# rvl-lab-utoronto/video_similarity_search

Measured on AMD Instinct MI355X. Metric: clips/sec R3D-18+NCE (1/2/4/8 GPU); k-means embeddings/sec 100k×512, higher is better.
Workload: dtype f32; 1 GPU; R3D-18 (3D-ResNet-18, 34.52 M params, no maxpool, 7^3 stem) fwd+bwd + NT-Xent (noise_contrastive, T=0.5) + SGD(lr .1, mom .5); per-GPU batch 32 x 3x16x112x112 fp32 = 16 anchors || 16 positives; BASELINE configs[1]; global_batch=32, parallelism=dp1

## Files before the change

include/slic_hip.h:

```cpp
#ifndef SLIC_HIP_H
#define SLIC_HIP_H

#include <stddef.h>
#include <stdint.h>

#ifdef __cplusplus
extern "C" {
#endif

#define SLIC_OK 0
#define SLIC_EINVAL -1
#define SLIC_EHIP -2
#define SLIC_ENODEV -3
#define SLIC_ETIMEOUT -4

int slic_version(void);
const char* slic_last_error(void);
int slic_device_check(void);


int slic_kmeans_cnorm(const float* C, int K, int D, int ldc, float* cnorm, void* stream);

size_t slic_kmeans_assign_workspace_bytes(int64_t N, int K);
int slic_kmeans_assign(const float* X, int64_t N, int D, int ldx, const float* C, int K, int ldc,
// ... 131 lines not shown
int slic_conv_gemm(const SlicConvArgs* args, int variant, void* stream);
int slic_conv_gemm_multi(const SlicConvArgs* args, int n, int variant, void* stream);
size_t slic_conv_gemm_tailsplit_workspace_bytes(const SlicConvArgs* args, int variant, int nfull_rb, int splits);
int slic_conv_gemm_tailsplit(const SlicConvArgs* args, int variant, int nfull_rb, int splits, void* workspace, void* stream);

size_t slic_conv_wgrad_workspace_bytes(const SlicConvArgs* args, int splits);
int slic_conv_wgrad(const SlicConvArgs* args, const float* dy, int ldy, int splits, int C, int ntaps,
                    float* dW, void* workspace, void* stream);
int slic_conv_row_table(const SlicConvArgs* args, uint32_t* row_tab, void* stream);
int slic_pack_weight_fwd(const float* W, int N, int C, int ntaps, int Cs, int Kp, float* Wp, void* stream);
int slic_pack_weight_fwd_runs(const float* W, int N, int C, int ntaps, int run_len, int run_px, int Kp, float* Wp, void* stream);
int slic_pack_weight_dgrad(const float* W, int N, int C, int ntaps, int Cs, int Kd, float* Wd, void* stream);
int slic_pack_weight_wino(const float* W, int N, int C, int dgrad, float* U, void* stream);
int slic_pack_weight_wino2(const float* W, int N, int C, int dgrad, float* U, void* stream);
size_t slic_conv_wgrad_wino2_workspace_bytes(const SlicConvArgs* args, int splits);
int slic_conv_wino2_tile_table(const SlicConvArgs* args, uint32_t* tile_tab, void* stream);
int slic_conv_wgrad_wino2(const SlicConvArgs* args, const float* dy, int splits, const uint32_t* tile_tab, float* dW,
                          void* workspace, void* stream);
size_t slic_conv_wgrad_wino_workspace_bytes(const SlicConvArgs* args, int splits);
int slic_conv_wino_tile_table(const SlicConvArgs* args, uint32_t* tile_tab, void* stream);
int slic_conv_wgrad_wino(const SlicConvArgs* args, const float* dy, int splits, const uint32_t* tile_tab, float* dW,
                         void* workspace, void* stream);
int slic_ncdhw_to_ndhwc(const float* x, int B, int C, int64_t S, int Cp, float* y, void* stream);
int slic_ncdhw_to_ndhwc_wpad(const float* x, int B, int C, int64_t R, int W, int pad_left, int Wp, float* y, void* stream);

int slic_pack_weight_stem_dgrad(const float* W, int N, int C, int kt, float* Wp, void* stream);
int slic_conv_stem_dgrad(const float* dz, const float* Wp, int B, int C, int T, int H, int W, int N, int kt, int st, float* dx,
                         void* stream);

int slic_bn_merge_stats(const float* partial, int R, int rows, int C, int64_t M, double* stats, void* workspace, void* stream);
// ... 174 lines not shown
```

video_similarity_search_amd/_lib.py:

```python
import ctypes
import os

import torch

_HERE = os.path.dirname(os.path.abspath(__file__))
LIB_PATH = os.environ.get("SLIC_LIB_PATH") or os.path.join(_HERE, "csrc", "libslic_hip.so")

c_void_p, c_int, c_int64, c_size_t, c_float, c_double = (
    ctypes.c_void_p, ctypes.c_int, ctypes.c_int64, ctypes.c_size_t, ctypes.c_float, ctypes.c_double)
P, I, L, F, Dbl = c_void_p, c_int, c_int64, c_float, c_double

SIGNATURES = {
    "slic_version": (I, []),
    "slic_last_error": (ctypes.c_char_p, []),
    "slic_device_check": (I, []),
    "slic_kmeans_cnorm": (I, [P, I, I, I, P, P]),
    "slic_kmeans_assign_workspace_bytes": (c_size_t, [L, I]),
    "slic_kmeans_assign": (I, [P, L, I, I, P, I, I, P, P, P, P, P, P, P]),
    "slic_kmeans_accumulate_workspace_bytes": (c_size_t, [L, I]),
    "slic_kmeans_accumulate": (I, [P, L, I, I, P, I, P, P, P, P]),
    "slic_kmeans_combine_shards": (I, [P, P, L, I, I, I, P, P, P]),
    "slic_kmeans_dist_to_assigned": (I, [P, L, I, I, P, I, P, P, P]),
    "slic_sum_f32_to_f64_workspace_bytes": (c_size_t, [L]),
    "slic_sum_f32_to_f64": (I, [P, L, P, P, P]),
# ... 36 lines not shown
    "slic_cumsum_search": (I, [P, L, P, I, P, P, P]),
    "slic_conv_tile_m": (I, [P, I]),
    "slic_conv_gemm": (I, [P, I, P]),
    "slic_conv_gemm_multi": (I, [P, I, I, P]),
    "slic_conv_gemm_tailsplit_workspace_bytes": (c_size_t, [P, I, I, I]),
    "slic_conv_gemm_tailsplit": (I, [P, I, I, I, P, P]),
    "slic_conv_wgrad_workspace_bytes": (c_size_t, [P, I]),
    "slic_conv_row_table": (I, [P, P, P]),
    "slic_conv_wgrad": (I, [P, P, I, I, I, I, P, P, P]),
    "slic_pack_weight_fwd": (I, [P, I, I, I, I, I, P, P]),
    "slic_pack_weight_fwd_runs": (I, [P, I, I, I, I, I, I, P, P]),
    "slic_pack_weight_dgrad": (I, [P, I, I, I, I, I, P, P]),
    "slic_pack_weight_wino": (I, [P, I, I, I, P, P]),
    "slic_pack_weight_wino2": (I, [P, I, I, I, P, P]),
    "slic_conv_wgrad_wino2_workspace_bytes": (c_size_t, [P, I]),
    "slic_conv_wino2_tile_table": (I, [P, P, P]),
    "slic_conv_wgrad_wino2": (I, [P, P, I, P, P, P, P]),
    "slic_conv_wgrad_wino_workspace_bytes": (c_size_t, [P, I]),
    "slic_conv_wino_tile_table": (I, [P, P, P]),
    "slic_conv_wgrad_wino": (I, [P, P, I, P, P, P, P]),
    "slic_ncdhw_to_ndhwc": (I, [P, I, I, L, I, P, P]),
    "slic_ncdhw_to_ndhwc_wpad": (I, [P, I, I, L, I, I, I, P, P]),
    "slic_pack_weight_stem_dgrad": (I, [P, I, I, I, P, P]),
    "slic_conv_stem_dgrad": (I, [P, P, I, I, I, I, I, I, I, I, P, P]),
    "slic_bn_finalize_workspace_bytes": (c_size_t, [I, I]),
    "slic_bn_finalize": (I, [P, I, I, I, L, F, F, P, P, P, P, P, P, P, P, P, P]),
    "slic_bn_eval_affine": (I, [P, P, P, P, F, I, P, P, P]),
    "slic_bn_merge_stats": (I, [P, I, I, I, L, P, P, P]),
    "slic_bn_finalize_sync": (I, [P, I, I, F, F, P, P, P, P, P, P, P, P, P]),
    "slic_bn_bwd_sums_workspace_bytes": (c_size_t, [L, I, I]),
# ... 175 lines not shown
```

video_similarity_search_amd/csrc/common.h:

```cpp
#pragma once
#include <hip/hip_runtime.h>
#include <stdint.h>
#include <stdio.h>
#include "../../include/slic_hip.h"

typedef float f32x4 __attribute__((ext_vector_type(4)));
typedef float f32x16 __attribute__((ext_vector_type(16)));
typedef int i32x4 __attribute__((ext_vector_type(4)));

void slic_set_error(const char* fmt, ...);

#define SLIC_REQUIRE(cond, ...)                 \
  do {                                          \
    if (!(cond)) {                              \
      slic_set_error(__VA_ARGS__);              \
      return SLIC_EINVAL;                       \
    }                                           \
  } while (0)

#define SLIC_HIP_CHECK(expr)                                                        \
  do {                                                                              \
    hipError_t _e = (expr);                                                         \
    if (_e != hipSuccess) {                                                         \
      slic_set_error("%s:%d: %s -> %s", __FILE__, __LINE__, #expr, hipGetErrorString(_e)); \
      return SLIC_EHIP;                                                             \
    }                                                                               \
  } while (0)

#define SLIC_LAUNCH_CHECK() SLIC_HIP_CHECK(hipGetLastError())

int slic_lds_limit(const void* kernel, size_t bytes);
int slic_device_cus(void);

#define SLIC_LDS_LIMIT(kernel, bytes)                                  \
  do {                                                                 \
    int _rc = slic_lds_limit((const void*)(kernel), (size_t)(bytes));  \
    if (_rc != SLIC_OK) return _rc;                                    \
  } while (0)

static inline hipStream_t S_(void* s) { return (hipStream_t)s; }

static inline size_t slic_align_up(size_t x, size_t a) { return (x + a - 1) / a * a; }
static inline int64_t slic_cdiv(int64_t a, int64_t b) { return (a + b - 1) / b; }

struct SlicCarver {
  char* p;
  size_t off;
// ... 9 lines not shown
```

video_similarity_search_amd/csrc/common.hip:

```cpp
#include "common.h"
#include <stdarg.h>
#include <string.h>
#include <map>
#include <mutex>
#include <utility>

static thread_local char g_err[512] = "";

void slic_set_error(const char* fmt, ...) {
  va_list ap;
  va_start(ap, fmt);
  vsnprintf(g_err, sizeof(g_err), fmt, ap);
  va_end(ap);
}

extern "C" int slic_version(void) { return (0 << 16) | (1 << 8) | 0; }

extern "C" const char* slic_last_error(void) { return g_err; }

extern "C" int slic_device_check(void) {
  int dev = 0;
  hipDeviceProp_t prop;
  if (hipGetDevice(&dev) != hipSuccess || hipGetDeviceProperties(&prop, dev) != hipSuccess) {
    slic_set_error("no HIP device visible");
// ... 14 lines not shown
  if (bytes > 160 * 1024) {
    slic_set_error("slic_lds_limit: %zu bytes of dynamic LDS", bytes);
    return SLIC_EHIP;
  }
  int dev = 0;
  SLIC_HIP_CHECK(hipGetDevice(&dev));
  std::lock_guard<std::mutex> lock(g_dev_mu);
  const auto key = std::make_pair(dev, kernel);
  const auto it = g_lds_limit.find(key);
  if (it != g_lds_limit.end() && bytes <= it->second) return SLIC_OK;
  SLIC_HIP_CHECK(hipFuncSetAttribute(kernel, hipFuncAttributeMaxDynamicSharedMemorySize, (int)bytes));
  g_lds_limit[key] = bytes;
  return SLIC_OK;
}

int slic_device_cus(void) {
  int dev = 0, cus = 0;
  if (hipGetDevice(&dev) != hipSuccess) { (void)hipGetLastError(); return 0; }
  std::lock_guard<std::mutex> lock(g_dev_mu);
  auto it = g_cus.find(dev);
  if (it != g_cus.end()) return it->second;
  if (hipDeviceGetAttribute(&cus, hipDeviceAttributeMultiprocessorCount, dev) != hipSuccess || cus <= 0) { (void)hipGetLastError(); return 0; }
  g_cus[dev] = cus;
  return cus;
}
```

video_similarity_search_amd/csrc/conv.hip:

```cpp
#include "common.h"
#include "conv_common.h"
#include "conv_internal.h"
#include <type_traits>
#ifndef SLIC_WG_ILVQ
#define SLIC_WG_ILVQ 7
#endif
#ifndef SLIC_PRIO_EDGE
#define SLIC_PRIO_EDGE 3
#endif
#ifndef SLIC_ILVQ
#define SLIC_ILVQ 2
#endif
#include <stdlib.h>
#ifndef SLIC_GEMM0_WPE
#define SLIC_GEMM0_WPE 4
#endif

#ifdef SLIC_STAMPS
__device__ unsigned long long* slic_stamps_buf = nullptr;
extern "C" int slic_debug_set_stamps(unsigned long long* buf) {
  return hipMemcpyToSymbol(HIP_SYMBOL(slic_stamps_buf), &buf, sizeof(buf)) == hipSuccess ? 0 : -1;
}
#define SLIC_STAMP(wg, slot)                                                                              \
  do {                                                                                                   \
// ... 22 lines not shown
    const int n = n0 + col;
    const float bias = (p.bias && n < p.N) ? p.bias[n] : 0.f;
#pragma unroll
    for (int i = 0; i < TM; ++i)
#pragma unroll
      for (int g = 0; g < 16; ++g) {
        const int row = wm * WTM + i * 32 + (g & 3) + 8 * (g >> 2) + 4 * h;
        tile[row * BN + col] = acc[i][j][g] + bias;
      }
  }
  __syncthreads();
  conv_epilogue_rows<BM, BN>(p, lds, m0, n0, tid);
}

template <int BM, int BN, int WM, int WN>
__global__ __launch_bounds__(256) __attribute__((amdgpu_waves_per_eu(SLIC_GEMM0_WPE, SLIC_GEMM0_WPE))) void conv_gemm_kernel(const SlicConvArgs p) {
  extern __shared__ __attribute__((aligned(16))) float lds[];
  constexpr int WTM = BM / WM, WTN = BN / WN;
  constexpr int TM = WTM / 32, TN = WTN / 32;
  constexpr int AL = BM / 32, BL = BN / 32;
  static_assert(WM * WN == 4, "4 waves");
  float* As = lds;
  float* Bs = lds + 2 * BM * 32;

  const int tid = threadIdx.x, lane = tid & 63, wave = tid >> 6;
  const int wm = wave / WN, wn = wave % WN;
  const int64_t m0 = (int64_t)blockIdx.x * BM;
  const int n0 = blockIdx.y * BN;

  const int cq = tid & 7, srow = tid >> 3;
  const __amdgpu_buffer_rsrc_t rs_src = __builtin_amdgcn_make_buffer_rsrc((void*)p.src, 0, p.src_bytes, 0x00020000);
// ... 17 lines not shown
      for (int o = -3; o <= 3; ++o) {
        mk |= ((unsigned)(a0 + o) < (unsigned)p.Ts ? 1u : 0u) << (o + 3);
        mk |= ((unsigned)(b0 + o) < (unsigned)p.Hs ? 1u : 0u) << (7 + o + 3);
        mk |= ((unsigned)(c0 + o) < (unsigned)p.Ws ? 1u : 0u) << (14 + o + 3);
      }
      rmask[i] = mk;
    }
  }
  unsigned woff[BL];
#pragma unroll
  for (int i = 0; i < BL; ++i) {
    const int n = n0 + srow + 32 * i;
    woff[i] = n < p.N ? (unsigned)n * (unsigned)p.ldw * 4u : OOB;
  }
  i32x4 gA[2][AL], gB[2][BL];
  const int nk = p.nchunks >> 3;
  int4 e_next = nk > 0 ? ((const int4*)p.tab)[cq] : make_int4(0, -1, 0, 0);
  auto gload = [&](int kt, i32x4 (&ga)[AL], i32x4 (&gb)[BL]) {
    const int4 e = e_next;
    const unsigned tm = (unsigned)e.y;
    const unsigned dlt = (unsigned)e.x * 4u;
#pragma unroll
    for (int i = 0; i < AL; ++i) {
      const unsigned off = ((rmask[i] & tm) == tm) ? aoff[i] + dlt : OOB;
      ga[i] = __builtin_amdgcn_raw_buffer_load_b128(rs_src, (int)off, 0, 0);
    }
    const unsigned wc = e.y == -1 ? OOB : (unsigned)e.z * 4u;
#pragma unroll
    for (int i = 0; i < BL; ++i) {
      const unsigned off = (woff[i] == OOB || wc == OOB) ? OOB : woff[i] + wc;
      gb[i] = __builtin_amdgcn_raw_buffer_load_b128(rs_wgt, (int)off, 0, 0);
    }
// ... 31 lines not shown
        for (int i = 0; i < TM; ++i) a[nxt][i] = *(const f32x4*)&Ab[cv_off(wm * WTM + i * 32 + r, 2 * (q + 1) + h)];
#pragma unroll
        for (int j = 0; j < TN; ++j) b[nxt][j] = *(const f32x4*)&Bb[cv_off(wn * WTN + j * 32 + r, 2 * (q + 1) + h)];
      }
#pragma unroll
      for (int t = 0; t < 4; ++t)
#pragma unroll
        for (int i = 0; i < TM; ++i)
#pragma unroll
          for (int j = 0; j < TN; ++j)
            acc[i][j] = __builtin_amdgcn_mfma_f32_32x32x2f32(a[cur][i][t], b[cur][j][t], acc[i][j], 0, 0, 0);
      if (q < 3) __builtin_amdgcn_sched_group_barrier(0x100, TM + TN, 0);
      __builtin_amdgcn_sched_group_barrier(0x008, 4 * TM * TN, 0);
    }
  };
  if (nk > 0) {
    gload(0, gA[0], gB[0]);
    lwrite(0, gA[0], gB[0]);
    if (nk > 1) gload(1, gA[1], gB[1]);
  }
  __syncthreads();
  for (int kt0 = 0; kt0 < nk; kt0 += 2) {
#pragma unroll
    for (int half = 0; half < 2; ++half) {
      const int kt = kt0 + half;
      if (kt < nk) {
        if (kt + 2 < nk) gload(kt + 2, gA[half], gB[half]);
        compute(half);
        if (kt + 1 < nk) lwrite(half ^ 1, gA[half ^ 1], gB[half ^ 1]);
        __syncthreads();
      }
    }
  }

  conv_epilogue<BM, BN, WM, WN, TM, TN>(p, acc, lds, m0, n0, wm, wn, r, h, tid);
}

// ... 1226 lines not shown
  }
  if (a->dst)
    SLIC_REQUIRE(a->N % 4 == 0 && a->ldo % 4 == 0 && ((uintptr_t)a->dst % 16) == 0 && (!a->addend || ((uintptr_t)a->addend % 16) == 0),
                 "%s: N and ldo must be multiples of 4 and dst / addend 16-byte aligned", who);
  SLIC_REQUIRE(((uintptr_t)a->src % 16) == 0, "%s: src not 16-byte aligned", who);
  SLIC_REQUIRE(a->src_bytes > 0 && a->src_bytes < 0xFFFFFF00u, "%s: src_bytes must be set and < 4 GiB (split the batch)", who);
  return SLIC_OK;
}

template <int BM, int BN, int WM, int WN>
static int launch_gemm(const SlicConvArgs& a, hipStream_t st) {
  constexpr size_t ring = (size_t)2 * (BM + BN) * 32 * sizeof(float), epi = (size_t)conv_epi_lds_floats(BM, BN) * sizeof(float);
  constexpr size_t lds = ring > epi ? ring : epi;
  SLIC_LDS_LIMIT((conv_gemm_kernel<BM, BN, WM, WN>), lds);
  dim3 grid((unsigned)slic_cdiv(a.M, BM), (unsigned)slic_cdiv(a.N, BN));
  conv_gemm_kernel<BM, BN, WM, WN><<<grid, dim3(256), lds, st>>>(a);
  SLIC_LAUNCH_CHECK();
  return SLIC_OK;
}

template <int BM, int BN, int WM, int WN, int STAGES = 2, int KD = 32>
static int launch_gemm_dma(const SlicConvArgs& a, hipStream_t st) {
  constexpr size_t ring = (size_t)STAGES * (BM + BN) * KD * sizeof(float), epi = (size_t)conv_epi_lds_floats(BM, BN) * sizeof(float);
  constexpr size_t lds = ring > epi ? ring : epi;
  SLIC_LDS_LIMIT((conv_gemm_dma_kernel<BM, BN, WM, WN, STAGES, KD>), lds);
  const unsigned gx = (unsigned)slic_cdiv(a.M, BM);
  dim3 grid((gx + 7) / 8 * 8, (unsigned)slic_cdiv(a.N, BN));
  conv_gemm_dma_kernel<BM, BN, WM, WN, STAGES, KD><<<grid, dim3(256), lds, st>>>(a, 1, nullptr, 0);
  SLIC_LAUNCH_CHECK();
  return SLIC_OK;
}
// ... 321 lines not shown
```

video_similarity_search_amd/csrc/conv_wino2.hip:

```cpp
#include "common.h"
#include "conv_epilogue.h"
#include "conv_internal.h"
#include "wino_common.h"
#include <type_traits>
#include <stdlib.h>

#ifndef SLIC_PRIO_EDGE
#define SLIC_PRIO_EDGE 3
#endif
#ifndef SLIC_W2_ABL
#define SLIC_W2_ABL 0
#endif
#ifdef SLIC_W2_STAMPS
__device__ unsigned long long* slic_w2_stamps_buf = nullptr;
extern "C" int slic_debug_set_w2_stamps(unsigned long long* buf) {
  return hipMemcpyToSymbol(HIP_SYMBOL(slic_w2_stamps_buf), &buf, sizeof(buf)) == hipSuccess ? 0 : -1;
}
#define W2_STAMP(slot)                                                                                                         \
  do {                                                                                                                         \
    if (threadIdx.x == 0 && slic_w2_stamps_buf)                                                                                \
      slic_w2_stamps_buf[(size_t)(blockIdx.x + gridDim.x * blockIdx.y) * 16 + (slot)] = __builtin_amdgcn_s_memrealtime();      \
  } while (0)
#define W2_STAMP_ID()                                                                                                          \
  do {                                                                                                                         \
// ... 1176 lines not shown
  SLIC_LAUNCH_CHECK();
  SLIC_LDS_LIMIT(conv_wino2_finish, lds);
  conv_wino2_finish<<<dim3((unsigned)tail, ny), dim3(512), lds, st>>>(*a, full, slab, nfull, pieces);
  SLIC_LAUNCH_CHECK();
  return SLIC_OK;
}

extern "C" int slic_pack_weight_wino2(const float* W, int N, int C, int dgrad, float* U, void* stream) {
  SLIC_REQUIRE(W && U && N % 64 == 0 && C % 64 == 0, "slic_pack_weight_wino2: N and C must be multiples of 64");
  const int64_t tot = (int64_t)3 * C * N;
  pack_w_wino2<<<dim3((unsigned)slic_cdiv(tot, 256)), dim3(256), 0, (hipStream_t)stream>>>(W, N, C, dgrad, U);
  SLIC_LAUNCH_CHECK();
  return SLIC_OK;
}

__global__ void conv_wino2_tile_table_kernel(const SlicConvArgs p, uint2* __restrict__ tab) {
  const int Wq = (p.Ws + 3) >> 2, Hq = (p.Hs + 1) >> 1;
  const int64_t tile = (int64_t)blockIdx.x * blockDim.x + threadIdx.x;
  if (tile >= (p.M / ((int64_t)p.Hs * p.Ws)) * Hq * Wq) return;
  unsigned q = (unsigned)tile;
  const int wt = (int)(q % (unsigned)Wq); q /= (unsigned)Wq;
  const int h2 = (int)(q % (unsigned)Hq); q /= (unsigned)Hq;
  const int tt = (int)(q % (unsigned)p.Ts);
  unsigned mk = 1u << 27;
#pragma unroll
  for (int a = 0; a < 4; ++a)
#pragma unroll
    for (int b = 0; b < 6; ++b) {
      const bool in = (unsigned)(2 * h2 - 1 + a) < (unsigned)p.Hs && (unsigned)(4 * wt - 1 + b) < (unsigned)p.Ws;
      mk |= (in ? 0u : 1u) << (a * 6 + b);
    }
#pragma unroll
  for (int kt = 0; kt < 3; ++kt) mk |= ((unsigned)(tt + kt - 1) < (unsigned)p.Ts ? 0u : 1u) << (24 + kt);
  tab[tile] = make_uint2((unsigned)(((int64_t)q * p.Hs + 2 * h2) * p.Ws + 4 * wt), mk);
}

constexpr int WB_TILE_BYTES = 8192;
constexpr int WB_STAGE_BYTES = 4 * WB_TILE_BYTES;
#ifndef SLIC_WB_STAGES
#define SLIC_WB_STAGES 4
#endif
constexpr int WB_STAGES = SLIC_WB_STAGES;

__global__ __launch_bounds__(512) __attribute__((amdgpu_waves_per_eu(2, 2)))
void conv_wgrad_wino2_kernel(const SlicConvArgs p, const float* __restrict__ dy, unsigned dy_bytes, const uint2* __restrict__ tile_tab,
                              float* __restrict__ slab, int tiles_per_split, int nsplit) {
  extern __shared__ __attribute__((aligned(16))) float lds[];
  const int tid = threadIdx.x, lane = tid & 63;
  const int wave = __builtin_amdgcn_readfirstlane(tid >> 6);
  const int j = wave & 3, wc = wave >> 2;
  const int r = lane & 31, hh = lane >> 5;
  const int C = p.Cs, N = p.N, H = p.Hs, W = p.Ws;
  const int CB = C >> 6, NBk = N >> 6;
  const int per_slice = 3 * CB * NBk;
  const int bx = blockIdx.x, gdx = gridDim.x;
  const int v = (bx & 7) * (gdx >> 3) + (bx >> 3);
  if (v >= per_slice * nsplit) return;
  const int z = v / per_slice;
  int rest = v - z * per_slice;
  const int kt = rest / (CB * NBk); rest -= kt * (CB * NBk);
  const int cb = rest / NBk, nb = rest - cb * NBk;
  const int Wq = (W + 3) >> 2, Hq = (H + 1) >> 1;
  const int64_t Mt = (p.M / ((int64_t)H * W)) * Hq * Wq;
  const int64_t tbeg = (int64_t)z * tiles_per_split;
  const int64_t tend = min(tbeg + tiles_per_split, Mt);
  const int nst = tend > tbeg ? (int)((tend - tbeg + 3) / 4) : 0;
  __builtin_amdgcn_s_setprio(SLIC_PRIO_EDGE);
  const __amdgpu_buffer_rsrc_t rs_src = __builtin_amdgcn_make_buffer_rsrc((void*)p.src, 0, p.src_bytes, 0x00020000);
  const int dt = wave >> 1, dh = wave & 1;
  const int sub = lane >> 4, chunk = lane & 15;
  const unsigned B0x = (unsigned)((((kt == 0 ? H * W : 0) + W + 1) * C) * 4);
  const __amdgpu_buffer_rsrc_t rs_23 = __builtin_amdgcn_make_buffer_rsrc(dh ? (void*)dy : (void*)p.src, 0, dh ? (int)dy_bytes : (int)p.src_bytes, 0x00020000);
  const unsigned pitch23 = (unsigned)((dh ? N : C) * 4), bias23 = dh ? 0u : B0x;
  unsigned cstb[4];
  int spos[4];
#pragma unroll
  for (int i = 0; i < 4; ++i) {
    const int d = 4 * dh + i;
    if (d >= 6) {
      const int hp = d - 6, o = sub;
// ... 165 lines not shown
    mfma_pts(cur, 3, 6);
    issue_tile(slotn, recn, 2);
    recn = load_rec(sg + WB_STAGES);
    transform_y(yf, ys, prev);
  };
  for (int s0 = 0; s0 < nst; s0 += WB_STAGES) {
    stage(s0, std::integral_constant<int, 0>{});
    stage(s0 + 1, std::integral_constant<int, 1>{});
    stage(s0 + 2, std::integral_constant<int, 2>{});
    stage(s0 + 3, std::integral_constant<int, 3>{});
    if constexpr (WB_STAGES == 5) stage(s0 + 4, std::integral_constant<int, 4>{});
  }
  mfma_pts(prev, 0, 6);
  asm volatile("s_waitcnt vmcnt(0)" ::: "memory");
  __builtin_amdgcn_s_setprio(SLIC_PRIO_EDGE);
  float* out = slab + (((int64_t)z * 3 + kt) * 4 + j) * 3 * (int64_t)C * N + nb * 64 + 2 * r;
#pragma unroll
  for (int g = 0; g < 16; ++g) {
    const int c = cb * 64 + 32 * wc + (g & 3) + 8 * (g >> 2) + 4 * hh;
    f32x2 t[3];
#pragma unroll
    for (int nh = 0; nh < 2; ++nh) {
      const float s12 = acc[1][nh][g] + acc[2][nh][g], d12 = acc[2][nh][g] - acc[1][nh][g];
      const float s34 = acc[3][nh][g] + acc[4][nh][g], d34 = acc[3][nh][g] - acc[4][nh][g];
      t[0][nh] = 0.25f * acc[0][nh][g] - (1.f / 6.f) * s12 + (1.f / 24.f) * s34;
      t[1][nh] = (1.f / 6.f) * d12 + (1.f / 12.f) * d34;
      t[2][nh] = -(1.f / 6.f) * s12 + (1.f / 6.f) * s34 + acc[5][nh][g];
    }
#pragma unroll
    for (int kw = 0; kw < 3; ++kw) *(f32x2*)(out + ((int64_t)kw * C + c) * N) = t[kw];
  }
}

template <int G>
__global__ __launch_bounds__(256) void conv_wgrad_wino2_reduce(const float* __restrict__ slab, int64_t gstride, int C, int N, float* __restrict__ dW) {
  __shared__ float outs[32 * 217];
  const int tid = threadIdx.x;
  const int nl = tid & 31, cl = tid >> 5;
  const int c0 = blockIdx.x * 8, n0 = blockIdx.y * 32;
  const int n = n0 + nl, c = c0 + cl;
  const int64_t CN = (int64_t)C * N;
#pragma unroll
  for (int kt = 0; kt < 3; ++kt) {
    float v[4][3][G];
#pragma unroll
    for (int jj = 0; jj < 4; ++jj)
#pragma unroll
      for (int kw = 0; kw < 3; ++kw) {
        const float* q = slab + (((int64_t)kt * 4 + jj) * 3 + kw) * CN + (int64_t)c * N + n;
#pragma unroll
        for (int g = 0; g < G; ++g) v[jj][kw][g] = q[g * gstride];
      }
    float t[4][3];
#pragma unroll
    for (int jj = 0; jj < 4; ++jj)
#pragma unroll
      for (int kw = 0; kw < 3; ++kw) {
        float a = v[jj][kw][0];
#pragma unroll
        for (int g = 1; g < G; ++g) a += v[jj][kw][g];
        t[jj][kw] = a;
      }
    float* o = outs + nl * 217 + cl * 27 + kt * 9;
#pragma unroll
    for (int kw = 0; kw < 3; ++kw) {
      const float h12 = 0.5f * (t[1][kw] - t[2][kw]);
      o[0 * 3 + kw] = t[0][kw] + h12;
      o[1 * 3 + kw] = 0.5f * (t[1][kw] + t[2][kw]);
      o[2 * 3 + kw] = h12 - t[3][kw];
    }
  }
  __syncthreads();
  for (int i = tid; i < 32 * 216; i += 256) {
    const int row = i / 216, e = i - row * 216;
    dW[((int64_t)(n0 + row) * C + c0) * 27 + e] = outs[row * 217 + e];
// ... 31 lines not shown
  const int p = (int)slic_cdiv(S, 8) < 8 ? 8 : (int)slic_cdiv(S, 8);
  *per = p;
  *G = (int)slic_cdiv(S, p);
}

static int64_t wino2_tiles(const SlicConvArgs* a) { return (a->M / ((int64_t)a->Hs * a->Ws)) * ((a->Hs + 1) / 2) * ((a->Ws + 3) / 4); }

static void wino2_wgrad_plan(const SlicConvArgs* a, int splits, int* tps, int* S) {
  const int64_t Mt = wino2_tiles(a);
  int64_t per = slic_cdiv(Mt, splits < 1 ? 1 : splits);
  per = slic_cdiv(per, 8) * 8;
  *tps = (int)per;
  *S = (int)slic_cdiv(Mt, per);
}

extern "C" size_t slic_conv_wgrad_wino2_workspace_bytes(const SlicConvArgs* a, int splits) {
  if (!a || a->M <= 0) return 0;
  int tps, S;
  wino2_wgrad_plan(a, splits, &tps, &S);
  return slic_align_up((size_t)S * 3 * 12 * a->Cs * a->N * sizeof(float), 256);
}

extern "C" int slic_conv_wino2_tile_table(const SlicConvArgs* a, uint32_t* tile_tab, void* stream) {
  SLIC_REQUIRE(a && tile_tab && a->M > 0 && a->Ws > 0 && a->Hs > 0 && a->Ga == a->Ts && a->Gb == a->Hs && a->Gc == a->Ws && a->Cs > 0,
               "slic_conv_wino2_tile_table: needs a stride-1 same-size geometry");
  SLIC_REQUIRE(a->M < (1ll << 24), "slic_conv_wino2_tile_table: more than 2^24 output positions (split the batch)");
  conv_wino2_tile_table_kernel<<<dim3((unsigned)slic_cdiv(wino2_tiles(a), 256)), dim3(256), 0, (hipStream_t)stream>>>(*a, (uint2*)tile_tab);
  SLIC_LAUNCH_CHECK();
  return SLIC_OK;
}

extern "C" int slic_conv_wgrad_wino2(const SlicConvArgs* a, const float* dy, int splits, const uint32_t* tile_tab, float* dW,
                                     void* workspace, void* stream) {
  SLIC_REQUIRE(a && a->src && dy && dW && workspace && tile_tab && splits >= 1, "slic_conv_wgrad_wino2: bad args");
  SLIC_REQUIRE(a->Cs % 64 == 0 && a->N % 64 == 0 && a->sa == 1 && a->sb == 1 && a->sc == 1 && a->Ga == a->Ts && a->Gb == a->Hs &&
                   a->Gc == a->Ws && !a->k_run_len,
               "slic_conv_wgrad_wino2: needs a 3x3x3 stride-1 same-size geometry, Cs %% 64 == 0, N %% 64 == 0");
  const int64_t dyb = a->M * (int64_t)a->N * 4;
  SLIC_REQUIRE(dyb < (int64_t)0xFFFFFF00u && a->M * (int64_t)a->Cs * 4 < (int64_t)0xFFFFFF00u && a->M < (1ll << 24),
               "slic_conv_wgrad_wino2: tensors larger than 4 GiB / 2^24 positions (split the batch)");
  int tps, S;
  wino2_wgrad_plan(a, splits, &tps, &S);
  hipStream_t st = (hipStream_t)stream;
  constexpr size_t lds = (size_t)WB_STAGES * WB_STAGE_BYTES;
  static_assert(lds <= 160 * 1024, "LDS");
  SLIC_LDS_LIMIT(conv_wgrad_wino2_kernel, lds);
  const int64_t total = (int64_t)3 * (a->Cs / 64) * (a->N / 64) * S;
  SLIC_REQUIRE(total < (1ll << 30), "slic_conv_wgrad_wino2: grid too large");
  const unsigned gx = (unsigned)((total + 7) / 8 * 8);
  conv_wgrad_wino2_kernel<<<dim3(gx), dim3(512), lds, st>>>(*a, dy, (unsigned)dyb, (const uint2*)tile_tab, (float*)workspace, tps, S);
  SLIC_LAUNCH_CHECK();
#if SLIC_W2_ABL & 4096
  return SLIC_OK;
#endif
  int per, G;
  wino2_wgrad_groups(S, &per, &G);
  const int64_t n4 = (int64_t)36 * a->Cs * a->N / 4;
  if (per > 1) {
    conv_wgrad_wino2_sum<<<dim3((unsigned)slic_cdiv(n4, 256), (unsigned)G), dim3(256), 0, st>>>((float*)workspace, S, per, n4);
    SLIC_LAUNCH_CHECK();
  }
  const dim3 rg((unsigned)(a->Cs / 8), (unsigned)(a->N / 32));
  const int64_t gstride = (int64_t)per * n4 * 4;
  switch (G) {
#define W2_RED(g) case g: conv_wgrad_wino2_reduce<g><<<rg, dim3(256), 0, st>>>((const float*)workspace, gstride, a->Cs, a->N, dW); break;
    W2_RED(1) W2_RED(2) W2_RED(3) W2_RED(4) W2_RED(5) W2_RED(6) W2_RED(7) W2_RED(8)
#undef W2_RED
    default: SLIC_REQUIRE(false, "slic_conv_wgrad_wino2: %d partial slabs", G);
  }
  SLIC_LAUNCH_CHECK();
  return SLIC_OK;
}
```

video_similarity_search_amd/models/conv_plan.py:

```python
import ctypes
import itertools
import os

import numpy as np
import torch

from .. import _lib
from .._lib import SlicConvArgs, call, ptr, stream


def _pad8(n):
    return (n + 7) // 8 * 8


def _pack_off(oa, ob, oc):
    assert -128 <= oa < 128 and -128 <= ob < 128 and -128 <= oc < 128
    return (oa + 128) | ((ob + 128) << 8) | ((oc + 128) << 16)


_ENV_KEYS = {}


def _env_fast_path():
    data = getattr(os.environ, "_data", None)
# ... 583 lines not shown
        if chunks is not None:
            tmp = torch.empty_like(dW)
            for i, (b0, b1) in enumerate(chunks):
                self.wgrad(x[b0:b1], dz[b0:b1], b1 - b0, dW if i == 0 else tmp, splits)
                if i:
                    dW.add_(tmp)
            return dW
        COUNTS["wgrad"] += 1
        a = self._fwd_args(x, B)
        if self.wino2_wgrad:
            blocks = 3 * (self.C // 64) * (self.N // 64)
            H2, W2 = self.in_dims[1], self.in_dims[2]
            mt = (a.M // (H2 * W2)) * ((H2 + 1) // 2) * ((W2 + 3) // 4)
            if splits is None:
                forced = _env("SLIC_WINO2_WGRAD_WGS")
                splits = max(1, min((int(forced) if forced else 256) // blocks, mt // 64))
            tab = self._wino2_tabs.get(B)
            if tab is None:
                tab = torch.empty(mt, 2, dtype=torch.int32, device=self.device)
                call("slic_conv_wino2_tile_table", ctypes.byref(a), ptr(tab), stream())
                self._wino2_tabs[B] = tab
            ws = _lib.workspace(lib.slic_conv_wgrad_wino2_workspace_bytes(ctypes.byref(a), splits), x.device, "wgrad")
            call("slic_conv_wgrad_wino2", ctypes.byref(a), ptr(dz), splits, ptr(tab), ptr(dW), ptr(ws), stream())
            return dW
        if self.wino_wgrad:
            blocks = 9 * (self.C // 64) * (self.N // 64)
            mt = (a.M // self.in_dims[2]) * ((self.in_dims[2] + 3) // 4)
            if splits is None:
                splits = self._wino_wgrad_slices(blocks, mt)
            tab = self._wino_tabs.get(B)
            if tab is None:
                tab = torch.empty(mt, 2, dtype=torch.int32, device=self.device)
                call("slic_conv_wino_tile_table", ctypes.byref(a), ptr(tab), stream())
                self._wino_tabs[B] = tab
            ws = _lib.workspace(lib.slic_conv_wgrad_wino_workspace_bytes(ctypes.byref(a), splits), x.device, "wgrad")
            call("slic_conv_wgrad_wino", ctypes.byref(a), ptr(dz), splits, ptr(tab), ptr(dW), ptr(ws), stream())
# ... 9 lines not shown
```

Baseline: 890.9 clips/s.

## Skip temporally padded K-chunks in conv GEMM and per-tap wino2 wgrad splits

The conv GEMM kernel now computes, per block, the range of K-chunks whose temporal taps touch live (non-padded) rows and iterates only over that range, which avoids loading and multiplying chunks that would be fully masked. For short time dimensions, the wino2 weight-gradient tile table is reordered time-major so that the outer temporal taps can skip the first or last time slice. The split count is then planned separately per tap, with a matching per-tap reduction. This adds a ballot/scan prologue to every GEMM block and more complex split planning, and it is gated by an environment variable whose default is 1, so the GEMM skip is on and the time-major wgrad path is off by default.

```diff
diff --git a/include/slic_hip.h b/include/slic_hip.h
--- a/include/slic_hip.h
+++ b/include/slic_hip.h
@@ -169,6 +169,7 @@
 int slic_pack_weight_wino(const float* W, int N, int C, int dgrad, float* U, void* stream);
 int slic_pack_weight_wino2(const float* W, int N, int C, int dgrad, float* U, void* stream);
 size_t slic_conv_wgrad_wino2_workspace_bytes(const SlicConvArgs* args, int splits);
+int slic_conv_wgrad_wino2_plan(const SlicConvArgs* args, int splits, int* out );
 int slic_conv_wino2_tile_table(const SlicConvArgs* args, uint32_t* tile_tab, void* stream);
 int slic_conv_wgrad_wino2(const SlicConvArgs* args, const float* dy, int splits, const uint32_t* tile_tab, float* dW,
                           void* workspace, void* stream);
diff --git a/video_similarity_search_amd/_lib.py b/video_similarity_search_amd/_lib.py
--- a/video_similarity_search_amd/_lib.py
+++ b/video_similarity_search_amd/_lib.py
@@ -74,6 +74,7 @@
     "slic_pack_weight_wino": (I, [P, I, I, I, P, P]),
     "slic_pack_weight_wino2": (I, [P, I, I, I, P, P]),
     "slic_conv_wgrad_wino2_workspace_bytes": (c_size_t, [P, I]),
+    "slic_conv_wgrad_wino2_plan": (I, [P, I, P]),
     "slic_conv_wino2_tile_table": (I, [P, P, P]),
     "slic_conv_wgrad_wino2": (I, [P, P, I, P, P, P, P]),
     "slic_conv_wgrad_wino_workspace_bytes": (c_size_t, [P, I]),
diff --git a/video_similarity_search_amd/csrc/common.h b/video_similarity_search_amd/csrc/common.h
--- a/video_similarity_search_amd/csrc/common.h
+++ b/video_similarity_search_amd/csrc/common.h
@@ -31,6 +31,7 @@
 
 int slic_lds_limit(const void* kernel, size_t bytes);
 int slic_device_cus(void);
+int slic_tpad_skip(void);
 
 #define SLIC_LDS_LIMIT(kernel, bytes)                                  \
   do {                                                                 \
diff --git a/video_similarity_search_amd/csrc/common.hip b/video_similarity_search_amd/csrc/common.hip
--- a/video_similarity_search_amd/csrc/common.hip
+++ b/video_similarity_search_amd/csrc/common.hip
@@ -1,5 +1,6 @@
 #include "common.h"
 #include <stdarg.h>
+#include <stdlib.h>
 #include <string.h>
 #include <map>
 #include <mutex>
@@ -52,6 +53,12 @@
   return SLIC_OK;
 }
 
+int slic_tpad_skip(void) {
+  const char* e = getenv("SLIC_TPAD_SKIP");
+  const int v = e ? atoi(e) : 1;
+  return v < 0 ? 0 : v > 2 ? 2 : v;
+}
+
 int slic_device_cus(void) {
   int dev = 0, cus = 0;
   if (hipGetDevice(&dev) != hipSuccess) { (void)hipGetLastError(); return 0; }
diff --git a/video_similarity_search_amd/csrc/conv.hip b/video_similarity_search_amd/csrc/conv.hip
--- a/video_similarity_search_amd/csrc/conv.hip
+++ b/video_similarity_search_amd/csrc/conv.hip
@@ -60,7 +60,7 @@
 }
 
 template <int BM, int BN, int WM, int WN>
-__global__ __launch_bounds__(256) __attribute__((amdgpu_waves_per_eu(SLIC_GEMM0_WPE, SLIC_GEMM0_WPE))) void conv_gemm_kernel(const SlicConvArgs p) {
+__global__ __launch_bounds__(256) __attribute__((amdgpu_waves_per_eu(SLIC_GEMM0_WPE, SLIC_GEMM0_WPE))) void conv_gemm_kernel(const SlicConvArgs p, const int tskip) {
   extern __shared__ __attribute__((aligned(16))) float lds[];
   constexpr int WTM = BM / WM, WTN = BN / WN;
   constexpr int TM = WTM / 32, TN = WTN / 32;
@@ -108,8 +108,43 @@
     woff[i] = n < p.N ? (unsigned)n * (unsigned)p.ldw * 4u : OOB;
   }
   i32x4 gA[2][AL], gB[2][BL];
-  const int nk = p.nchunks >> 3;
-  int4 e_next = nk > 0 ? ((const int4*)p.tab)[cq] : make_int4(0, -1, 0, 0);
+  int k_lo = 0, nk = p.nchunks >> 3;
+  if (tskip) {
+    __shared__ unsigned sh_u[4];
+    __shared__ int sh_k[4][2];
+    unsigned tb = 0;
+#pragma unroll
+    for (int i = 0; i < AL; ++i) tb |= rmask[i] & 0x7Fu;
+    unsigned wu = 0;
+#pragma unroll
+    for (int b = 0; b < 7; ++b) wu |= (__builtin_amdgcn_ballot_w64((tb >> b) & 1u) != 0ull ? 1u : 0u) << b;
+    if (lane == 0) sh_u[wave] = wu;
+    __syncthreads();
+    const unsigned U = sh_u[0] | sh_u[1] | sh_u[2] | sh_u[3];
+    int lo = nk, hi = 0;
+    for (int c0 = 0; c0 < p.nchunks; c0 += 256) {
+      const int c = c0 + tid;
+      bool live = false;
+      if (c < p.nchunks) {
+        const unsigned y = (unsigned)((const int4*)p.tab)[c].y;
+        live = y != 0xFFFFFFFFu && (y & 0x7Fu & ~U) == 0u;
+      }
+      const unsigned long long bm = __builtin_amdgcn_ballot_w64(live);
+      if (bm) {
+        const int c_w = c0 + wave * 64;
+        lo = min(lo, (c_w + __builtin_ctzll(bm)) >> 3);
+        hi = max(hi, ((c_w + 63 - __builtin_clzll(bm)) >> 3) + 1);
+      }
+    }
+    if (lane == 0) { sh_k[wave][0] = lo; sh_k[wave][1] = hi; }
+    __syncthreads();
+    lo = min(min(sh_k[0][0], sh_k[1][0]), min(sh_k[2][0], sh_k[3][0]));
+    hi = max(max(sh_k[0][1], sh_k[1][1]), max(sh_k[2][1], sh_k[3][1]));
+    lo = __builtin_amdgcn_readfirstlane(lo);
+    hi = __builtin_amdgcn_readfirstlane(hi);
+    if (hi > lo) { k_lo = lo; nk = hi; } else nk = 0;
+  }
+  int4 e_next = nk > k_lo ? ((const int4*)p.tab)[k_lo * 8 + cq] : make_int4(0, -1, 0, 0);
   auto gload = [&](int kt, i32x4 (&ga)[AL], i32x4 (&gb)[BL]) {
     const int4 e = e_next;
     const unsigned tm = (unsigned)e.y;
@@ -171,13 +206,13 @@
       __builtin_amdgcn_sched_group_barrier(0x008, 4 * TM * TN, 0);
     }
   };
-  if (nk > 0) {
-    gload(0, gA[0], gB[0]);
+  if (nk > k_lo) {
+    gload(k_lo, gA[0], gB[0]);
     lwrite(0, gA[0], gB[0]);
-    if (nk > 1) gload(1, gA[1], gB[1]);
+    if (nk > k_lo + 1) gload(k_lo + 1, gA[1], gB[1]);
   }
   __syncthreads();
-  for (int kt0 = 0; kt0 < nk; kt0 += 2) {
+  for (int kt0 = k_lo; kt0 < nk; kt0 += 2) {
 #pragma unroll
     for (int half = 0; half < 2; ++half) {
       const int kt = kt0 + half;
@@ -1434,7 +1469,7 @@
   constexpr size_t lds = ring > epi ? ring : epi;
   SLIC_LDS_LIMIT((conv_gemm_kernel<BM, BN, WM, WN>), lds);
   dim3 grid((unsigned)slic_cdiv(a.M, BM), (unsigned)slic_cdiv(a.N, BN));
-  conv_gemm_kernel<BM, BN, WM, WN><<<grid, dim3(256), lds, st>>>(a);
+  conv_gemm_kernel<BM, BN, WM, WN><<<grid, dim3(256), lds, st>>>(a, a.k_run_len > 0 && slic_tpad_skip() >= 1);
   SLIC_LAUNCH_CHECK();
   return SLIC_OK;
 }
diff --git a/video_similarity_search_amd/csrc/conv_wino2.hip b/video_similarity_search_amd/csrc/conv_wino2.hip
--- a/video_similarity_search_amd/csrc/conv_wino2.hip
+++ b/video_similarity_search_amd/csrc/conv_wino2.hip
@@ -1214,14 +1214,19 @@
   return SLIC_OK;
 }
 
-__global__ void conv_wino2_tile_table_kernel(const SlicConvArgs p, uint2* __restrict__ tab) {
+__global__ void conv_wino2_tile_table_kernel(const SlicConvArgs p, uint2* __restrict__ tab, int tmajor) {
   const int Wq = (p.Ws + 3) >> 2, Hq = (p.Hs + 1) >> 1;
   const int64_t tile = (int64_t)blockIdx.x * blockDim.x + threadIdx.x;
   if (tile >= (p.M / ((int64_t)p.Hs * p.Ws)) * Hq * Wq) return;
   unsigned q = (unsigned)tile;
   const int wt = (int)(q % (unsigned)Wq); q /= (unsigned)Wq;
   const int h2 = (int)(q % (unsigned)Hq); q /= (unsigned)Hq;
-  const int tt = (int)(q % (unsigned)p.Ts);
+  int tt = (int)(q % (unsigned)p.Ts);
+  if (tmajor) {
+    const unsigned Bn = (unsigned)(p.M / ((int64_t)p.Ts * p.Hs * p.Ws));
+    tt = (int)(q / Bn);
+    q = (q - (unsigned)tt * Bn) * (unsigned)p.Ts + (unsigned)tt;
+  }
   unsigned mk = 1u << 27;
 #pragma unroll
   for (int a = 0; a < 4; ++a)
@@ -1234,6 +1239,8 @@
   for (int kt = 0; kt < 3; ++kt) mk |= ((unsigned)(tt + kt - 1) < (unsigned)p.Ts ? 0u : 1u) << (24 + kt);
   tab[tile] = make_uint2((unsigned)(((int64_t)q * p.Hs + 2 * h2) * p.Ws + 4 * wt), mk);
 }
+
+struct W2WgDeal { int S[3], tps[3], beg[3], end[3], perkt; };
 
 constexpr int WB_TILE_BYTES = 8192;
 constexpr int WB_STAGE_BYTES = 4 * WB_TILE_BYTES;
@@ -1244,7 +1251,7 @@
 
 __global__ __launch_bounds__(512) __attribute__((amdgpu_waves_per_eu(2, 2)))
 void conv_wgrad_wino2_kernel(const SlicConvArgs p, const float* __restrict__ dy, unsigned dy_bytes, const uint2* __restrict__ tile_tab,
-                              float* __restrict__ slab, int tiles_per_split, int nsplit) {
+                              float* __restrict__ slab, const W2WgDeal dl) {
   extern __shared__ __attribute__((aligned(16))) float lds[];
   const int tid = threadIdx.x, lane = tid & 63;
   const int wave = __builtin_amdgcn_readfirstlane(tid >> 6);
@@ -1252,18 +1259,24 @@
   const int r = lane & 31, hh = lane >> 5;
   const int C = p.Cs, N = p.N, H = p.Hs, W = p.Ws;
   const int CB = C >> 6, NBk = N >> 6;
-  const int per_slice = 3 * CB * NBk;
+  const int blk = CB * NBk;
   const int bx = blockIdx.x, gdx = gridDim.x;
   const int v = (bx & 7) * (gdx >> 3) + (bx >> 3);
-  if (v >= per_slice * nsplit) return;
-  const int z = v / per_slice;
-  int rest = v - z * per_slice;
-  const int kt = rest / (CB * NBk); rest -= kt * (CB * NBk);
+  if (v >= blk * (dl.S[0] + dl.S[1] + dl.S[2])) return;
+  int sl, kt, z, rest;
+  if (dl.perkt) {
+    sl = v / blk; rest = v - sl * blk;
+    kt = sl < dl.S[0] ? 0 : sl < dl.S[0] + dl.S[1] ? 1 : 2;
+    z = sl - (kt == 0 ? 0 : kt == 1 ? dl.S[0] : dl.S[0] + dl.S[1]);
+  } else {
+    z = v / (3 * blk); rest = v - z * 3 * blk;
+    kt = rest / blk; rest -= kt * blk;
+    sl = z * 3 + kt;
+  }
   const int cb = rest / NBk, nb = rest - cb * NBk;
-  const int Wq = (W + 3) >> 2, Hq = (H + 1) >> 1;
-  const int64_t Mt = (p.M / ((int64_t)H * W)) * Hq * Wq;
-  const int64_t tbeg = (int64_t)z * tiles_per_split;
-  const int64_t tend = min(tbeg + tiles_per_split, Mt);
+  const int tps = kt == 0 ? dl.tps[0] : kt == 1 ? dl.tps[1] : dl.tps[2];
+  const int64_t tbeg = (kt == 0 ? dl.beg[0] : kt == 1 ? dl.beg[1] : dl.beg[2]) + (int64_t)z * tps;
+  const int64_t tend = min(tbeg + tps, (int64_t)(kt == 0 ? dl.end[0] : kt == 1 ? dl.end[1] : dl.end[2]));
   const int nst = tend > tbeg ? (int)((tend - tbeg + 3) / 4) : 0;
   __builtin_amdgcn_s_setprio(SLIC_PRIO_EDGE);
   const __amdgpu_buffer_rsrc_t rs_src = __builtin_amdgcn_make_buffer_rsrc((void*)p.src, 0, p.src_bytes, 0x00020000);
@@ -1459,7 +1472,7 @@
   mfma_pts(prev, 0, 6);
   asm volatile("s_waitcnt vmcnt(0)" ::: "memory");
   __builtin_amdgcn_s_setprio(SLIC_PRIO_EDGE);
-  float* out = slab + (((int64_t)z * 3 + kt) * 4 + j) * 3 * (int64_t)C * N + nb * 64 + 2 * r;
+  float* out = slab + ((int64_t)sl * 4 + j) * 3 * (int64_t)C * N + nb * 64 + 2 * r;
 #pragma unroll
   for (int g = 0; g < 16; ++g) {
     const int c = cb * 64 + 32 * wc + (g & 3) + 8 * (g >> 2) + 4 * hh;
@@ -1477,8 +1490,10 @@
   }
 }
 
-template <int G>
-__global__ __launch_bounds__(256) void conv_wgrad_wino2_reduce(const float* __restrict__ slab, int64_t gstride, int C, int N, float* __restrict__ dW) {
+struct W2RedKt { int64_t ktoff[3]; int cnt[3]; };
+template <int G, bool PERKT>
+__global__ __launch_bounds__(256) void conv_wgrad_wino2_reduce(const float* __restrict__ slab, int64_t gstride, const W2RedKt rk, int C, int N,
+                                                               float* __restrict__ dW) {
   __shared__ float outs[32 * 217];
   const int tid = threadIdx.x;
   const int nl = tid & 31, cl = tid >> 5;
@@ -1487,14 +1502,15 @@
   const int64_t CN = (int64_t)C * N;
 #pragma unroll
   for (int kt = 0; kt < 3; ++kt) {
+    const int cnt = PERKT ? rk.cnt[kt] : G;
     float v[4][3][G];
 #pragma unroll
     for (int jj = 0; jj < 4; ++jj)
 #pragma unroll
       for (int kw = 0; kw < 3; ++kw) {
-        const float* q = slab + (((int64_t)kt * 4 + jj) * 3 + kw) * CN + (int64_t)c * N + n;
-#pragma unroll
-        for (int g = 0; g < G; ++g) v[jj][kw][g] = q[g * gstride];
+        const float* q = slab + (PERKT ? rk.ktoff[kt] : (int64_t)kt * 12 * CN) + ((int64_t)jj * 3 + kw) * CN + (int64_t)c * N + n;
+#pragma unroll
+        for (int g = 0; g < G; ++g) v[jj][kw][g] = g < cnt ? q[g * gstride] : 0.f;
       }
     float t[4][3];
 #pragma unroll
@@ -1503,7 +1519,8 @@
       for (int kw = 0; kw < 3; ++kw) {
         float a = v[jj][kw][0];
 #pragma unroll
-        for (int g = 1; g < G; ++g) a += v[jj][kw][g];
+        for (int g = 1; g < G; ++g)
+          if (g < cnt) a += v[jj][kw][g];
         t[jj][kw] = a;
       }
     float* o = outs + nl * 217 + cl * 27 + kt * 9;
@@ -1565,56 +1582,132 @@
   *S = (int)slic_cdiv(Mt, per);
 }
 
+static int wino2_table_tmajor(const SlicConvArgs* a) { return slic_tpad_skip() >= 2 && a->Ts <= 4; }
+
+static void wino2_wgrad_deal(const SlicConvArgs* a, int splits, W2WgDeal* dl) {
+  const int64_t Mt = wino2_tiles(a);
+  const int blk = (a->Cs / 64) * (a->N / 64);
+  int cus = slic_device_cus();
+  if (!cus) cus = 256;
+  const int T = a->Ts;
+  if (wino2_table_tmajor(a) && blk > 0) {
+    const int64_t live[2] = {T > 1 ? Mt - Mt / T : 0, Mt};
+    const int budget = splits >= 1 ? splits : cus / blk;
+    int64_t cap[2];
+    for (int i = 0; i < 2; ++i) cap[i] = live[i] == 0 ? 0 : splits >= 1 ? slic_cdiv(live[i], 8) : live[i] / 64 < 1 ? 1 : live[i] / 64;
+    auto per_of = [](int64_t n, int64_t sl) { return sl ? slic_cdiv(slic_cdiv(n, sl), 8) * 8 : (int64_t)0; };
+    int best0 = -1, best1 = -1;
+    int64_t best = 0;
+    for (int s0 = live[0] ? 1 : 0; s0 <= cap[0] && 2 * s0 < budget; ++s0) {
+      const int64_t s1 = budget - 2 * s0 < cap[1] ? budget - 2 * s0 : cap[1];
+      const int64_t p0 = per_of(live[0], s0), p1 = per_of(live[1], s1), worst = p0 > p1 ? p0 : p1;
+      if (best0 < 0 || worst < best) { best0 = s0; best1 = (int)s1; best = worst; }
+    }
+    while (best0 >= 0 && best1 > 1 && per_of(live[1], best1 - 1) <= best) --best1;
+    if (best0 > 8 || best1 > 8) best0 = -1;
+    if (best0 >= 0) {
+      const int s[3] = {best0, best1, best0};
+      const int64_t beg[3] = {T > 1 ? Mt / T : 0, 0, 0}, end[3] = {T > 1 ? Mt : 0, Mt, T > 1 ? Mt - Mt / T : 0};
+      for (int kt = 0; kt < 3; ++kt) {
+        const int64_t n = end[kt] - beg[kt], per = per_of(n, s[kt]);
+        dl->tps[kt] = (int)per;
+        dl->S[kt] = per ? (int)slic_cdiv(n, per) : 0;
+        dl->beg[kt] = (int)beg[kt];
+        dl->end[kt] = (int)end[kt];
+      }
+      dl->perkt = 1;
+      return;
+    }
+  }
+  if (splits < 1) {
+    const int64_t s = cus / (3 * (blk > 0 ? blk : 1)), m = Mt / 64;
+    splits = (int)(s < m ? s : m);
+  }
+  int tps, S;
+  wino2_wgrad_plan(a, splits, &tps, &S);
+  for (int kt = 0; kt < 3; ++kt) { dl->S[kt] = S; dl->tps[kt] = tps; dl->beg[kt] = 0; dl->end[kt] = (int)Mt; }
+  dl->perkt = 0;
+}
+
+extern "C" int slic_conv_wgrad_wino2_plan(const SlicConvArgs* a, int splits, int* out) {
+  SLIC_REQUIRE(a && out && a->M > 0 && a->Ts > 0 && a->Hs > 0 && a->Ws > 0 && a->Cs >= 64 && a->N >= 64 && splits >= 0 &&
+                   wino2_tiles(a) < (1ll << 24),
+               "slic_conv_wgrad_wino2_plan: bad args");
+  W2WgDeal dl;
+  wino2_wgrad_deal(a, splits, &dl);
+  out[0] = wino2_table_tmajor(a);
+  out[1] = dl.perkt;
+  for (int kt = 0; kt < 3; ++kt) { out[2 + kt] = dl.S[kt]; out[5 + kt] = dl.tps[kt]; }
+  out[8] = (dl.S[0] + dl.S[1] + dl.S[2]) * (a->Cs / 64) * (a->N / 64);
+  return SLIC_OK;
+}
+
 extern "C" size_t slic_conv_wgrad_wino2_workspace_bytes(const SlicConvArgs* a, int splits) {
   if (!a || a->M <= 0) return 0;
-  int tps, S;
-  wino2_wgrad_plan(a, splits, &tps, &S);
-  return slic_align_up((size_t)S * 3 * 12 * a->Cs * a->N * sizeof(float), 256);
+  W2WgDeal dl;
+  wino2_wgrad_deal(a, splits, &dl);
+  return slic_align_up((size_t)(dl.S[0] + dl.S[1] + dl.S[2]) * 12 * a->Cs * a->N * sizeof(float), 256);
 }
 
 extern "C" int slic_conv_wino2_tile_table(const SlicConvArgs* a, uint32_t* tile_tab, void* stream) {
   SLIC_REQUIRE(a && tile_tab && a->M > 0 && a->Ws > 0 && a->Hs > 0 && a->Ga == a->Ts && a->Gb == a->Hs && a->Gc == a->Ws && a->Cs > 0,
                "slic_conv_wino2_tile_table: needs a stride-1 same-size geometry");
   SLIC_REQUIRE(a->M < (1ll << 24), "slic_conv_wino2_tile_table: more than 2^24 output positions (split the batch)");
-  conv_wino2_tile_table_kernel<<<dim3((unsigned)slic_cdiv(wino2_tiles(a), 256)), dim3(256), 0, (hipStream_t)stream>>>(*a, (uint2*)tile_tab);
+  conv_wino2_tile_table_kernel<<<dim3((unsigned)slic_cdiv(wino2_tiles(a), 256)), dim3(256), 0, (hipStream_t)stream>>>(*a, (uint2*)tile_tab,
+                                                                                                                        wino2_table_tmajor(a));
   SLIC_LAUNCH_CHECK();
   return SLIC_OK;
 }
 
 extern "C" int slic_conv_wgrad_wino2(const SlicConvArgs* a, const float* dy, int splits, const uint32_t* tile_tab, float* dW,
                                      void* workspace, void* stream) {
-  SLIC_REQUIRE(a && a->src && dy && dW && workspace && tile_tab && splits >= 1, "slic_conv_wgrad_wino2: bad args");
+  SLIC_REQUIRE(a && a->src && dy && dW && workspace && tile_tab && splits >= 0, "slic_conv_wgrad_wino2: bad args");
   SLIC_REQUIRE(a->Cs % 64 == 0 && a->N % 64 == 0 && a->sa == 1 && a->sb == 1 && a->sc == 1 && a->Ga == a->Ts && a->Gb == a->Hs &&
                    a->Gc == a->Ws && !a->k_run_len,
                "slic_conv_wgrad_wino2: needs a 3x3x3 stride-1 same-size geometry, Cs %% 64 == 0, N %% 64 == 0");
   const int64_t dyb = a->M * (int64_t)a->N * 4;
   SLIC_REQUIRE(dyb < (int64_t)0xFFFFFF00u && a->M * (int64_t)a->Cs * 4 < (int64_t)0xFFFFFF00u && a->M < (1ll << 24),
                "slic_conv_wgrad_wino2: tensors larger than 4 GiB / 2^24 positions (split the batch)");
-  int tps, S;
-  wino2_wgrad_plan(a, splits, &tps, &S);
+  W2WgDeal dl;
+  wino2_wgrad_deal(a, splits, &dl);
   hipStream_t st = (hipStream_t)stream;
   constexpr size_t lds = (size_t)WB_STAGES * WB_STAGE_BYTES;
   static_assert(lds <= 160 * 1024, "LDS");
   SLIC_LDS_LIMIT(conv_wgrad_wino2_kernel, lds);
-  const int64_t total = (int64_t)3 * (a->Cs / 64) * (a->N / 64) * S;
+  const int64_t total = (int64_t)(a->Cs / 64) * (a->N / 64) * (dl.S[0] + dl.S[1] + dl.S[2]);
   SLIC_REQUIRE(total < (1ll << 30), "slic_conv_wgrad_wino2: grid too large");
   const unsigned gx = (unsigned)((total + 7) / 8 * 8);
-  conv_wgrad_wino2_kernel<<<dim3(gx), dim3(512), lds, st>>>(*a, dy, (unsigned)dyb, (const uint2*)tile_tab, (float*)workspace, tps, S);
+  conv_wgrad_wino2_kernel<<<dim3(gx), dim3(512), lds, st>>>(*a, dy, (unsigned)dyb, (const uint2*)tile_tab, (float*)workspace, dl);
   SLIC_LAUNCH_CHECK();
 #if SLIC_W2_ABL & 4096
   return SLIC_OK;
 #endif
+  const int64_t n4 = (int64_t)36 * a->Cs * a->N / 4;
+  const dim3 rg((unsigned)(a->Cs / 8), (unsigned)(a->N / 32));
+  W2RedKt rk = {};
+  if (dl.perkt) {
+    const int64_t one = n4 * 4 / 3;
+    rk.ktoff[0] = 0; rk.ktoff[1] = dl.S[0] * one; rk.ktoff[2] = (dl.S[0] + dl.S[1]) * one;
+    for (int kt = 0; kt < 3; ++kt) rk.cnt[kt] = dl.S[kt];
+    switch (dl.S[1] > dl.S[0] ? dl.S[1] : dl.S[0]) {
+#define W2_RED(g) case g: conv_wgrad_wino2_reduce<g, true><<<rg, dim3(256), 0, st>>>((const float*)workspace, one, rk, a->Cs, a->N, dW); break;
+      W2_RED(1) W2_RED(2) W2_RED(3) W2_RED(4) W2_RED(5) W2_RED(6) W2_RED(7) W2_RED(8)
+#undef W2_RED
+      default: SLIC_REQUIRE(false, "slic_conv_wgrad_wino2: per-kt deal of more than 8 slices");
+    }
+    SLIC_LAUNCH_CHECK();
+    return SLIC_OK;
+  }
+  const int S = dl.S[0];
   int per, G;
   wino2_wgrad_groups(S, &per, &G);
-  const int64_t n4 = (int64_t)36 * a->Cs * a->N / 4;
   if (per > 1) {
     conv_wgrad_wino2_sum<<<dim3((unsigned)slic_cdiv(n4, 256), (unsigned)G), dim3(256), 0, st>>>((float*)workspace, S, per, n4);
     SLIC_LAUNCH_CHECK();
   }
-  const dim3 rg((unsigned)(a->Cs / 8), (unsigned)(a->N / 32));
   const int64_t gstride = (int64_t)per * n4 * 4;
   switch (G) {
-#define W2_RED(g) case g: conv_wgrad_wino2_reduce<g><<<rg, dim3(256), 0, st>>>((const float*)workspace, gstride, a->Cs, a->N, dW); break;
+#define W2_RED(g) case g: conv_wgrad_wino2_reduce<g, false><<<rg, dim3(256), 0, st>>>((const float*)workspace, gstride, rk, a->Cs, a->N, dW); break;
     W2_RED(1) W2_RED(2) W2_RED(3) W2_RED(4) W2_RED(5) W2_RED(6) W2_RED(7) W2_RED(8)
 #undef W2_RED
     default: SLIC_REQUIRE(false, "slic_conv_wgrad_wino2: %d partial slabs", G);
diff --git a/video_similarity_search_amd/models/conv_plan.py b/video_similarity_search_amd/models/conv_plan.py
--- a/video_similarity_search_amd/models/conv_plan.py
+++ b/video_similarity_search_amd/models/conv_plan.py
@@ -621,12 +621,14 @@
             mt = (a.M // (H2 * W2)) * ((H2 + 1) // 2) * ((W2 + 3) // 4)
             if splits is None:
                 forced = _env("SLIC_WINO2_WGRAD_WGS")
-                splits = max(1, min((int(forced) if forced else 256) // blocks, mt // 64))
-            tab = self._wino2_tabs.get(B)
+                splits = max(1, min(int(forced) // blocks, mt // 64)) if forced else 0
+            wplan = (ctypes.c_int * 9)()
+            call("slic_conv_wgrad_wino2_plan", ctypes.byref(a), splits, wplan)
+            tab = self._wino2_tabs.get((B, wplan[0]))
             if tab is None:
                 tab = torch.empty(mt, 2, dtype=torch.int32, device=self.device)
                 call("slic_conv_wino2_tile_table", ctypes.byref(a), ptr(tab), stream())
-                self._wino2_tabs[B] = tab
+                self._wino2_tabs[(B, wplan[0])] = tab
             ws = _lib.workspace(lib.slic_conv_wgrad_wino2_workspace_bytes(ctypes.byref(a), splits), x.device, "wgrad")
             call("slic_conv_wgrad_wino2", ctypes.byref(a), ptr(dz), splits, ptr(tab), ptr(dW), ptr(ws), stream())
             return dW
```

Result: no change. 895.8 clips/s (median of 6 runs) (+0.5%).
